# graphdeco-inria/editable-gaussian-reflections

Measured on AMD Instinct MI355X. Metric: Mrays/s fwd+bwd @1080p, 1M Gaussians, higher is better.
Workload: dtype f32; 1 GPU; BASELINE config C: synthetic dense-init room+spheres cloud, HEADLINE variant = init (literal dense-init opacity 0.1 (config.py:44): Kc ~ 22 per ray, bounces mostly die), N=1000000, 1920x1080, one training iteration: export + update_bvh + forward + backward + grad import, num_bounces=2, jitter on, reference default config; variant=init, gaussians=1000000, width=1920, height=1080, parallelism=image tiles x1 + 1 all-reduce of the launch's [22N] gradients, team_help=product default (on)

## Files before the change

editable-gaussian-reflections_amd/csrc/backward_chain.inc:

```
    const int lane = threadIdx.x & (EGR_WAVE - 1);
    const int wv = __builtin_amdgcn_readfirstlane((int)(threadIdx.x >> 6));
    __shared__ uint32_t gt_keys_all[TEAM][EGR_GT_SLOTS];
    __shared__ __attribute__((aligned(16))) float gt_vals_all[TEAM][EGR_GT_STRIDE * EGR_GT_SLOTS];
    __shared__ uint32_t gt_claim_all[TEAM][EGR_GT_SLOTS];
    __shared__ float4 stage_all[TEAM][4 * EGR_WAVE];
    __shared__ BwdTeamShared<TEAM> bteam;
    uint32_t *const gt_keys = gt_keys_all[wv], *const gt_claim = gt_claim_all[wv];
    float *const gt_vals = gt_vals_all[wv];
    float4 *const stage = stage_all[wv];
    if (threadIdx.x == 0) bteam.done = 0u;
    if (threadIdx.x < TEAM) bteam.ticket[threadIdx.x] = 0u, bteam.nitems[threadIdx.x] = 0u, bteam.finished[threadIdx.x] = 0u;
    uint32_t bepoch = 0u;
#define EGR_BQ_FLOATS (25 * EGR_WAVE)
    static_assert(EGR_GT_STRIDE * EGR_GT_SLOTS >= EGR_BQ_FLOATS, "the bounce queues must fit into the table");
    uint4 *bitems = reinterpret_cast<uint4 *>(gt_vals);
    float *bdl = gt_vals + 16 * EGR_WAVE;
    float *bray = gt_vals + 19 * EGR_WAVE;
    for (int s = lane; s < EGR_GT_SLOTS; s += EGR_WAVE) gt_keys[s] = EGR_GT_EMPTY;
    for (int s = lane; s < EGR_GT_STRIDE * EGR_GT_SLOTS; s += EGR_WAVE) gt_vals[s] = 0.0f;
    __syncthreads();
    const float exp_power = *v.cfg.exp_power;
    const float eps_scale_grad = *v.cfg.eps_scale_grad;
    const int num_bounces = min(*v.cfg.num_bounces, EGR_MAX_BOUNCES);
    const float view_size = BATCH ? 0.0f : tanf(*v.cam.vertical_fov_radians / 2.0f);
    uint32_t cur_q = blockIdx.x & 7u;
    uint32_t records = 0u;

    for (;;) {
        const uint32_t tq = wave_next_task(v.queues + 8 * EGR_QUEUE_STRIDE, BATCH ? v.num_tasks * v.batch_frames : v.num_tasks, cur_q, lane);
        if (tq == 0xFFFFFFFFu) break;
        EGR_TIMES(unsigned long long bw_t0 = 0ull, bw_t1 = 0ull; uint32_t bw_rows0 = 0u;) EGR_TIMES_IS(8, bw_t0 = __builtin_amdgcn_s_memrealtime();)
        bool table_dirty = false;
        {
            constexpr bool PRIMARY = true;
            const int step = 0;
            do {
#include "backward_task.inc"
// ... 10 lines not shown
            EGR_BWD_SYNC();
            for (int s = lane; s < EGR_BQ_FLOATS; s += EGR_WAVE) gt_vals[s] = 0.0f;
            EGR_BWD_SYNC();
        }
        EGR_TIMES_IS(8,
            const unsigned long long bw_t2 = __builtin_amdgcn_s_memrealtime();
            const uint32_t bt = v.bwd_order[tq];
            const TaskGeom btg = task_geom(v, BATCH ? batch_base_task(v, bt) : bt, lane);
            if (btg.inside) {
                if (lane == 0) v.stats.num_traversed_per_pixel[btg.pixel_id] = EGR_STAMP31(bw_t0), v.stats.num_accumulated_per_pixel[btg.pixel_id] = EGR_STAMP31(bw_t2);
                if (lane == 1) v.stats.num_traversed_per_pixel[btg.pixel_id] = EGR_STAMP31(bw_t1), v.stats.num_accumulated_per_pixel[btg.pixel_id] = (int32_t)bw_rows0;
            })
    }
    if constexpr (TEAM > 1) {
        if (lane == 0) atomicAdd(&bteam.done, 1u);
        records += bwd_team_help<TEAM>(v, exp_power, eps_scale_grad, bteam, gt_vals_all, stage, wv, lane);
    }
    if (lane == 0 && records) atomicAdd(v.control + CW_BUCKET_RECORDS, records);
```

editable-gaussian-reflections_amd/csrc/backward_task.inc:

```
        const uint32_t task = v.bwd_order[tq];
        uint32_t blk = v.task_last_block[(size_t)step * (BATCH ? v.num_tasks * v.batch_frames : v.num_tasks) + task];
        if (blk == 0xFFFFFFFFu) continue;
        uint32_t tb = task, bframe = 0u;
        if constexpr (BATCH) tb = batch_base_task(v, task), bframe = v.batch_frame0 + (task >> v.task_shift) % v.batch_frames;
        (void)bframe;
        const TaskGeom tg = task_geom(v, tb, lane);
        const StateRef S = state_of(v, task, lane);
        uint32_t steps_done = tg.inside ? f2u(S.ld(F_STEPS)) : 0u;
        uint32_t nhits = (tg.inside && (uint32_t)step < steps_done && blk != 0xFFFFFFFFu) ? f2u(S.ld(SF(step, S_NHITS))) : 0u;
        const uint32_t max_hits = wave_max_u32(nhits);
        if (max_hits == 0) continue;
        EGR_TIMES_IS(8, if (PRIMARY) bw_rows0 = max_hits;)

        f3 dL_rgb = mk3(0, 0, 0), dL_n = mk3(0, 0, 0), dL_f0 = mk3(0, 0, 0);
        float dL_depth = 0.0f, dL_rough = 0.0f;
        f3 ro = mk3(0, 0, 0), rd = mk3(0, 0, 1);
        f3 rem_rgb = mk3(0, 0, 0), rem_n = mk3(0, 0, 0), rem_f0 = mk3(0, 0, 0);
        float rem_depth = 0.0f, rem_rough = 0.0f, T_minus_Ttot = 0.0f;
        if (nhits > 0) {
            const uint32_t pid = tg.pixel_id;
            const float third = 1.0f / 3.0f;
            if (PRIMARY && BATCH) {
                f3 o_rgb = S.ld3(SF(0, S_RGB)), o_n = S.ld3(SF(0, S_NORMAL)), o_f0 = S.ld3(SF(0, S_F0));
                float o_depth = S.ld(SF(0, S_DEPTH)), o_rough = S.ld(SF(0, S_ROUGH));
// ... 34 lines not shown
                    const float *ts = v.fb.target_specular + 3 * (size_t)pid;
                    t_spec = mk3(ts[0], ts[1], ts[2]);
                }
                float down = powf(1.0f - S.ld(SF(step - 1, S_ROUGH)), EGR_ROUGHNESS_DOWNWEIGHT_GRAD_POWER);
                dL_rgb = (mk3(third * sign1(spec.x - t_spec.x), third * sign1(spec.y - t_spec.y), third * sign1(spec.z - t_spec.z)) *
                          *v.cfg.loss_weight_specular) * down;
                dL_rgb = dL_rgb * S.ld3(SF(step - 1, S_THR));
                ro = S.ld3(SF(step - 1, S_NEXT_O));
                rd = S.ld3(SF(step - 1, S_NEXT_D));
            }
            rem_rgb = S.ld3(SF(step, S_REM_RGB)), rem_n = S.ld3(SF(step, S_REM_NORMAL)), rem_f0 = S.ld3(SF(step, S_REM_F0));
            rem_depth = S.ld(SF(step, S_REM_DEPTH)), rem_rough = S.ld(SF(step, S_REM_ROUGH));
            T_minus_Ttot = S.ld(SF(step, S_T)) - S.ld(SF(step, S_TTOT));
        }

        auto hit_geometry = [&](uint32_t pos, const float4 &a2, const f3 &ro, const f3 &rd, float dL_dalpha, auto &gx) { hit_geometry_fn<true>(v, exp_power, eps_scale_grad, pos, a2, ro, rd, dL_dalpha, gx); };

        if constexpr (!PRIMARY) {
            table_dirty = true;
            bdl[lane] = dL_rgb.x, bdl[EGR_WAVE + lane] = dL_rgb.y, bdl[2 * EGR_WAVE + lane] = dL_rgb.z;
            bray[lane] = ro.x, bray[EGR_WAVE + lane] = ro.y, bray[2 * EGR_WAVE + lane] = ro.z, bray[3 * EGR_WAVE + lane] = rd.x, bray[4 * EGR_WAVE + lane] = rd.y, bray[5 * EGR_WAVE + lane] = rd.z;
            f3 prev_rgb = mk3(0, 0, 0), w_rgb = mk3(0, 0, 0);
            const uint32_t nblocks = (max_hits + EGR_HIT_BLOCK_ROWS - 1) / EGR_HIT_BLOCK_ROWS;
            EGR_BWD_SYNC();
            for (uint32_t b = nblocks; b-- > 0;) {
                const float4 *rows = v.hit_arena + (size_t)blk * (EGR_HIT_BLOCK_ROWS + 1) * EGR_WAVE;
                for (int chunk = EGR_HIT_BLOCK_ROWS / 4 - 1; chunk >= 0; chunk--) {
                    uint32_t nitems = 0u;
                    float4 rec4[4], a04[4];
#pragma unroll
                    for (int r4 = 0; r4 < 4; r4++) rec4[r4] = rows[(size_t)(1 + 4 * chunk + r4) * EGR_WAVE + lane];
// ... 29 lines not shown
                    EGR_BWD_SYNC();
                    const uint32_t nbatch = (nitems + (uint32_t)EGR_WAVE - 1u) / (uint32_t)EGR_WAVE;
                    if constexpr (TEAM > 1) {
                        if (lane == 0) {
                            lds_poke(&bteam.finished[wv], 0u);
                            lds_poke(&bteam.nitems[wv], nitems);
                            bepoch = (bepoch + 1u) & 0xFFFu;
                            lds_poke(&bteam.ticket[wv], (bepoch << 20) | (nbatch << 10));
                        }
                        for (;;) {
                            uint32_t tk = 0u;
                            if (lane == 0) tk = atomicAdd(&bteam.ticket[wv], 1u);
                            tk = uniform_u32(tk);
                            const uint32_t bi = tk & 0x3FFu;
                            if (bi >= nbatch) break;
                            records += bounce_batch(v, exp_power, eps_scale_grad, bitems, bdl, bray, bi * (uint32_t)EGR_WAVE, nitems, stage, lane);
                            if (lane == 0) atomicAdd(&bteam.finished[wv], 1u);
                        }
                        while (uniform_u32(lds_peek(&bteam.finished[wv])) < nbatch) __builtin_amdgcn_s_sleep(1);
                    } else {
                        for (uint32_t bi = 0; bi < nbatch; bi++) records += bounce_batch(v, exp_power, eps_scale_grad, bitems, bdl, bray, bi * (uint32_t)EGR_WAVE, nitems, stage, lane);
                    }
                    EGR_BWD_SYNC();
                }
                blk = f2u(rows[0].x);
            }
            continue;
        }
        f3 prev_rgb = mk3(0, 0, 0), w_rgb = mk3(0, 0, 0), prev_n = mk3(0, 0, 0), w_n = mk3(0, 0, 0), prev_f0 = mk3(0, 0, 0), w_f0 = mk3(0, 0, 0);
        float prev_rough = 0, w_rough = 0, prev_depth = 0, w_depth = 0;
        const uint32_t nblocks = (max_hits + EGR_HIT_BLOCK_ROWS - 1) / EGR_HIT_BLOCK_ROWS;
        EGR_STATS(unsigned long long bt_math = 0ull, bt_table = 0ull, bt_wide = 0ull, bt_rows = 0ull;)
        for (uint32_t b = nblocks; b-- > 0;) {
            const float4 *rows = v.hit_arena + (size_t)blk * (EGR_HIT_BLOCK_ROWS + 1) * EGR_WAVE;
            int pf_row = -1;
            float4 rec_pf = make_float4(0.f, 0.f, 0.f, 0.f);
// ... 54 lines not shown
                    dL_dalpha += tmp2 * dot(rem_f0, dL_f0);
                    dL_dalpha += tmp2 * (rem_rough * dL_rough);
                    dL_dalpha += tmp2 * (rem_depth * dL_depth);

                    hit_geometry(pos, a2, ro, rd, dL_dalpha, gx);
                    gx[PC_RGB] = d_rgb.x, gx[PC_RGB + 1] = d_rgb.y, gx[PC_RGB + 2] = d_rgb.z, gx[PC_WEIGHT] = weight;
                    gx[PC_NORMAL] = d_n.x, gx[PC_NORMAL + 1] = d_n.y, gx[PC_NORMAL + 2] = d_n.z;
                    gx[PC_F0] = d_f0.x, gx[PC_F0 + 1] = d_f0.y, gx[PC_F0 + 2] = d_f0.z, gx[PC_ROUGH] = d_rough;
                    EGR_STATS(bt1 = __builtin_amdgcn_s_memtime();)
                    dpos = pos;
                    want = primary_presum(pos, gx, lane);
                }
                direct = primary_table_add(v, want, dpos, gx, gt_keys, gt_vals, gt_claim, stage, lane, records);
                EGR_STATS(const unsigned long long bt2 = __builtin_amdgcn_s_memtime(); bt_math += bt1 - bt0; bt_table += bt2 - bt1;)
                if (__ballot(direct) != 0ull) {
                    float lo[15];
#pragma unroll
                    for (int c = 0; c < 15; c++) lo[c] = gx[c];
                    wide_add_wave<REC_PRIMARY_A>(v, direct, dpos, lo, stage);
                    float hi[15];
#pragma unroll
                    for (int c = 0; c < 15; c++) hi[c] = (15 + c < EGR_GT_COMPS) ? gx[(15 + c < EGR_GT_COMPS) ? 15 + c : 0] : 0.0f;
                    wide_add_wave<REC_PRIMARY_Q>(v, direct, dpos, hi, stage);
                    records += 2u * (uint32_t)__popcll(__ballot(direct));
                }
                EGR_STATS(bt_wide += __builtin_amdgcn_s_memtime() - bt2;)
            }
            blk = f2u(rows[0].x);
        }
        EGR_STATS(const unsigned long long bt3 = __builtin_amdgcn_s_memtime();)
        records += grad_table_flush(v, gt_keys, gt_vals, stage, lane);
        EGR_STATS(if (lane == 0) {
            unsigned long long *d = diag64(v.control, DG_BWD_MATH_CYC, !PRIMARY);
            atomicAdd(d, bt_math), atomicAdd(d + 1, bt_table), atomicAdd(d + 2, bt_wide), atomicAdd(d + 3, __builtin_amdgcn_s_memtime() - bt3), atomicAdd(d + 4, bt_rows);
        })
```

editable-gaussian-reflections_amd/csrc/trace.hip:

```cpp
#include <algorithm>
#include <cstdio>
#include <cstdlib>
#include <type_traits>
#include <utility>
#include <vector>

#define EGR_CONTRACT_AFTER_EPILOGUE
#include "egr_diag.hpp"
#include "egr_epilogue.hpp"

#ifndef EGR_GPOP
#define EGR_GPOP 5
#endif
#define EGR_WALK_MAX_LEAVES (8 * EGR_GPOP * EGR_WIDTH)
#define EGR_LBUF (64 + 2 * EGR_WALK_MAX_LEAVES)
#ifndef EGR_FPOP
#define EGR_FPOP 2
#endif
#ifndef EGR_PSTK
#define EGR_PSTK 512
#endif

namespace {

// ... 515 lines not shown
template <bool CUBE, int TEAM> __global__ void __launch_bounds__(EGR_WAVE * TEAM) __attribute__((amdgpu_waves_per_eu(EGR_FWD_WAVES, EGR_FWD_WAVES))) k_forward_batch(DeviceView v) {
    constexpr bool GRADS = false, BATCH = true;
#include "forward_chain.inc"
}
template <bool CUBE, int TEAM> __global__ void __launch_bounds__(EGR_WAVE * TEAM) __attribute__((amdgpu_waves_per_eu(EGR_FWD_WAVES, EGR_FWD_WAVES))) k_forward_batch_grads(DeviceView v) {
    constexpr bool GRADS = true, BATCH = true;
#include "forward_chain.inc"
}

#ifndef EGR_GT_SLOTS
#define EGR_GT_SLOTS 80
#endif
#define EGR_GT_COMPS 21
#define EGR_GT_STRIDE 21
#define EGR_GT_EMPTY 0xFFFFFFFFu
enum : int { GC_OPA = 0, GC_SCALE = 1, GC_MEAN = 4, GC_ROT = 7, GC_RGB = 11, GC_WEIGHT = 14, GC_NORMAL = 15, GC_F0 = 18, GC_ROUGH = 21, GC_Q = 22 };
enum : int { PC_OPA = 0, PC_MEAN = 1, PC_RGB = 4, PC_WEIGHT = 7, PC_NORMAL = 8, PC_F0 = 11, PC_ROUGH = 14, PC_Q = 15 };
enum : int { REC_BOUNCE = 0, REC_PRIMARY_A = 1, REC_PRIMARY_Q = 2 };
#define EGR_ROW_STRIDE 32
#define EGR_BWD_SYNC() wave_sync()

template <int REC> EGR_DI void wide_add_wave(const DeviceView &v, bool ok, uint32_t pos, const float (&r)[15], float4 *stage) {
    const int lane = threadIdx.x & (EGR_WAVE - 1);
    uint32_t cell = 0u;
    if constexpr (REC == REC_PRIMARY_A) {
        constexpr int cells[15] = {GC_OPA, GC_MEAN, GC_MEAN + 1, GC_MEAN + 2, GC_RGB, GC_RGB + 1, GC_RGB + 2, GC_WEIGHT, GC_NORMAL, GC_NORMAL + 1, GC_NORMAL + 2, GC_F0, GC_F0 + 1, GC_F0 + 2, GC_ROUGH};
#pragma unroll
        for (int i = 0; i < 15; i++) cell = (lane & 15) == i + 1 ? (uint32_t)cells[i] : cell;
    } else {
        cell = (REC == REC_PRIMARY_Q ? (uint32_t)GC_Q : 0u) + (uint32_t)((lane & 15) - 1);
    }
    if (ok) {
        stage[4 * lane + 0] = make_float4(u2f(pos), r[0], r[1], r[2]);
        stage[4 * lane + 1] = make_float4(r[3], r[4], r[5], r[6]);
        stage[4 * lane + 2] = make_float4(r[7], r[8], r[9], r[10]);
        stage[4 * lane + 3] = make_float4(r[11], r[12], r[13], r[14]);
    }
    const unsigned long long okm = __ballot(ok);
    EGR_BWD_SYNC();
    const float *sf = reinterpret_cast<const float *>(stage);
#pragma unroll 4
    for (int pass = 0; pass < 16; pass++) {
        const int src = 4 * pass + (lane >> 4), c = lane & 15;
        if (((okm >> (4 * pass)) & 0xFull) == 0ull) continue;
        const float x = sf[16 * src + c];
        const uint32_t p = f2u(sf[16 * src]);
        if (((okm >> src) & 1ull) && c != 0 && (REC != REC_PRIMARY_Q || c <= 6) && x != 0.0f) atomicAdd(v.grad_rows + (size_t)p * EGR_ROW_STRIDE + cell, x);
    }
    EGR_BWD_SYNC();
}

EGR_DI uint32_t grad_table_flush(const DeviceView &v, uint32_t *gt_keys, float *gt_vals, float4 *stage, int lane) {
    uint32_t sent = 0u;
    EGR_BWD_SYNC();
    for (int s0 = 0; s0 < EGR_GT_SLOTS; s0 += EGR_WAVE) {
        const int s = min(s0 + lane, EGR_GT_SLOTS - 1);
        const bool in_table = s0 + lane < EGR_GT_SLOTS;
        const uint32_t pos = in_table ? gt_keys[s] : EGR_GT_EMPTY;
        const bool valid = pos != EGR_GT_EMPTY;
        if (in_table) gt_keys[s] = EGR_GT_EMPTY;
        float lo[15], hi[15];
#pragma unroll
        for (int c = 0; c < 15; c++) {
            lo[c] = valid ? gt_vals[s * EGR_GT_STRIDE + c] : 0.0f;
            if (valid) gt_vals[s * EGR_GT_STRIDE + c] = 0.0f;
        }
#pragma unroll
        for (int c = 0; c < 15; c++) {
            hi[c] = 0.0f;
            if (15 + c < EGR_GT_COMPS) {
                hi[c] = valid ? gt_vals[s * EGR_GT_STRIDE + 15 + c] : 0.0f;
                if (valid) gt_vals[s * EGR_GT_STRIDE + 15 + c] = 0.0f;
            }
        }
        if (__ballot(valid) == 0ull) continue;
        wide_add_wave<REC_PRIMARY_A>(v, valid, pos, lo, stage);
        wide_add_wave<REC_PRIMARY_Q>(v, valid, pos, hi, stage);
        sent += 2u * (uint32_t)__popcll(__ballot(valid));
    }
    EGR_BWD_SYNC();
    return sent;
}

EGR_DI bool primary_presum(const uint32_t pos, float (&gx)[EGR_GT_COMPS], const int lane) {
    bool mine = true;
    {
        const unsigned long long em = __ballot(true);
#define EGR_FETCH_DPP(x, ctrl) __builtin_amdgcn_update_dpp(0, (int)(x), ctrl, 0xF, 0xF, false)
#define EGR_FETCH_SWZ(x, pat) __builtin_amdgcn_ds_swizzle((int)(x), pat)
#define EGR_FETCH_X32(x, unused) __shfl_xor((int)(x), 32)
#define EGR_FETCH_DPP4(x, unused) __builtin_amdgcn_update_dpp(0, __builtin_amdgcn_update_dpp(0, (int)(x), 0x141, 0xF, 0xF, false), 0x1B, 0xF, 0xF, false)
#define EGR_COMBINE(d, FETCH, arg)                                                                            \
// ... 45 lines not shown
        const bool win = pending && gt_claim[slot] == (uint32_t)lane;
        if (win) {
            float *cell = gt_vals + slot * EGR_GT_STRIDE;
            float cur[EGR_GT_COMPS];
#pragma unroll
            for (int c = 0; c < EGR_GT_COMPS; c++) cur[c] = cell[c];
#pragma unroll
            for (int c = 0; c < EGR_GT_COMPS; c++) cell[c] = cur[c] + gx[c];
            pending = false;
        }
        EGR_BWD_SYNC();
    }
    return want && !found;
}

template <class T> EGR_DI T chain_rcp(T b) {
    if constexpr (sizeof(T) == sizeof(float)) return egr_rcp_refined(b);
    else return T(1) / b;
}
template <class T> EGR_DI T chain_div(T a, T b, T r) {
    if constexpr (sizeof(T) == sizeof(float)) return egr_div_rn(a, b, r);
    else return a / b;
}
template <class T> EGR_DI T chain_sqrt(T x) {
    if constexpr (sizeof(T) == sizeof(float)) return egr_sqrt_rn(x);
    else return sqrt(x);
}
template <class T> struct ChainVec { T x, y, z; };
template <class T> EGR_DI void scale_rot_chain(const float4 &M0, const float4 &M1, const float4 &M2, const float4 &qu, const float sigma, const float eps, const ChainVec<T> &dl2w0,
                                               const ChainVec<T> &dl2w1, const ChainVec<T> &dl2w2, T (&d_scale)[3], T (&d_rot)[4]) {
    const T scaling_factor = sigma, eps_scale_grad = eps;
    const ChainVec<T> scaling = {T(M0.w), T(M1.w), T(M2.w)};
    const ChainVec<T> den = {scaling.x * scaling_factor + eps_scale_grad, scaling.y * scaling_factor + eps_scale_grad, scaling.z * scaling_factor + eps_scale_grad};
    const ChainVec<T> rden = {chain_rcp(den.x), chain_rcp(den.y), chain_rcp(den.z)};
    auto div3 = [&](const float4 &m) { return ChainVec<T>{chain_div(T(m.x), den.x, rden.x), chain_div(T(m.y), den.y, rden.y), chain_div(T(m.z), den.z, rden.z)}; };
    const ChainVec<T> rot_0 = div3(M0), rot_1 = div3(M1), rot_2 = div3(M2);
    d_scale[0] = (dl2w0.x * rot_0.x + dl2w1.x * rot_1.x + dl2w2.x * rot_2.x) * scaling.x;
    d_scale[1] = (dl2w0.y * rot_0.y + dl2w1.y * rot_1.y + dl2w2.y * rot_2.y) * scaling.y;
    d_scale[2] = (dl2w0.z * rot_0.z + dl2w1.z * rot_1.z + dl2w2.z * rot_2.z) * scaling.z;
    auto mul3 = [](const ChainVec<T> &a, const ChainVec<T> &b) { return ChainVec<T>{a.x * b.x, a.y * b.y, a.z * b.z}; };
    const ChainVec<T> dr0 = mul3(dl2w0, scaling), dr1 = mul3(dl2w1, scaling), dr2 = mul3(dl2w2, scaling);
    const T qr = qu.x, qx = qu.y, qy = qu.z, qz = qu.w;
    const T qn = chain_sqrt(qr * qr + qx * qx + qy * qy + qz * qz);
    const T rqn = chain_rcp(qn);
    const T r = chain_div(qr, qn, rqn), x = chain_div(qx, qn, rqn), y = chain_div(qy, qn, rqn), z = chain_div(qz, qn, rqn);
    const T dL_dr = T(2) * x * (dr2.y - dr1.z) + T(2) * y * (dr0.z - dr2.x) + T(2) * z * (dr1.x - dr0.y);
    const T dL_dx = T(-4) * x * (dr1.y + dr2.z) + T(2) * y * (dr0.y + dr1.x) + T(2) * z * (dr0.z + dr2.x) + T(2) * r * (dr2.y - dr1.z);
    const T dL_dy = T(2) * x * (dr0.y + dr1.x) - T(4) * y * (dr0.x + dr2.z) + T(2) * z * (dr1.z + dr2.y) + T(2) * r * (dr0.z - dr2.x);
    const T dL_dz = T(2) * x * (dr0.z + dr2.x) + T(2) * y * (dr1.z + dr2.y) - T(4) * z * (dr0.x + dr1.y) + T(2) * r * (dr1.x - dr0.y);
    const T dd = dL_dr * qr + dL_dx * qx + dL_dy * qy + dL_dz * qz;
    const T qn3 = qn * qn * qn;
    const T inv3 = chain_div(T(1), qn3, chain_rcp(qn3)), inv1 = chain_div(T(1), qn, rqn);
    d_rot[0] = dd * -qr * inv3 + dL_dr * inv1, d_rot[1] = dd * -qx * inv3 + dL_dx * inv1;
    d_rot[2] = dd * -qy * inv3 + dL_dy * inv1, d_rot[3] = dd * -qz * inv3 + dL_dz * inv1;
}

template <bool PRIMARY_HIT, class GX> EGR_DI void hit_geometry_fn(const DeviceView &v, const float exp_power, const float eps_scale_grad, uint32_t pos, const float4 &a2, const f3 &ro, const f3 &rd, float dL_dalpha, GX &gx) {
    const float opacity = a2.z, scaling_factor = a2.w;
    const float4 W0 = v.inst_w[4 * pos], W1 = v.inst_w[4 * pos + 1], W2 = v.inst_w[4 * pos + 2];
    float4 M0, M1, M2, qu;
    if constexpr (!PRIMARY_HIT) M0 = v.inst_m[4 * pos], M1 = v.inst_m[4 * pos + 1], M2 = v.inst_m[4 * pos + 2], qu = v.inst_m[4 * pos + 3];
    f3 lo, ld, dhat, u;
    float t_unused;
    bool behind_unused, outside_unused;
    candidate_geometry(W0, W1, W2, ro, rd, lo, ld, dhat, t_unused, u, behind_unused, outside_unused);
    const f3 local_hit = u * scaling_factor;
    const float sq_norm = dot(local_hit, local_hit);
    const float gaussval = egr_gaussian_sq(sq_norm, exp_power);

    float d_opacity = EGR_MAX_ALPHA * dL_dalpha * gaussval;
    d_opacity = d_opacity * opacity * (1.0f - opacity);
    const float dL_dgaussval = EGR_MAX_ALPHA * dL_dalpha * opacity;
    const float dL_dsq_norm = gaussval * pow_exp_m1(sq_norm, exp_power);
    const f3 dL_dx_local = (-local_hit * dL_dsq_norm) * dL_dgaussval;
    const f3 dL_dx_world = mk3(dot(mk3(W0.x, W1.x, W2.x), dL_dx_local), dot(mk3(W0.y, W1.y, W2.y), dL_dx_local),
                               dot(mk3(W0.z, W1.z, W2.z), dL_dx_local)) * scaling_factor;
    const f3 d_mean = -dL_dx_world;
    if constexpr (PRIMARY_HIT) {
        gx[PC_OPA] = d_opacity, gx[PC_MEAN] = d_mean.x, gx[PC_MEAN + 1] = d_mean.y, gx[PC_MEAN + 2] = d_mean.z;
        const f3 ql = -dL_dx_local * scaling_factor;
        gx[PC_Q] = ql.x * local_hit.x, gx[PC_Q + 1] = ql.x * local_hit.y, gx[PC_Q + 2] = ql.x * local_hit.z;
        gx[PC_Q + 3] = ql.y * local_hit.y, gx[PC_Q + 4] = ql.y * local_hit.z, gx[PC_Q + 5] = ql.z * local_hit.z;
    } else {
        const f3 dl2w0 = -dL_dx_world.x * local_hit, dl2w1 = -dL_dx_world.y * local_hit, dl2w2 = -dL_dx_world.z * local_hit;
        float d_scale[3], d_rot[4];
        scale_rot_chain<float>(M0, M1, M2, qu, scaling_factor, eps_scale_grad, {dl2w0.x, dl2w0.y, dl2w0.z}, {dl2w1.x, dl2w1.y, dl2w1.z}, {dl2w2.x, dl2w2.y, dl2w2.z}, d_scale, d_rot);
        gx[GC_OPA] = d_opacity, gx[GC_SCALE] = d_scale[0], gx[GC_SCALE + 1] = d_scale[1], gx[GC_SCALE + 2] = d_scale[2];
        gx[GC_MEAN] = d_mean.x, gx[GC_MEAN + 1] = d_mean.y, gx[GC_MEAN + 2] = d_mean.z;
        gx[GC_ROT] = d_rot[0], gx[GC_ROT + 1] = d_rot[1], gx[GC_ROT + 2] = d_rot[2], gx[GC_ROT + 3] = d_rot[3];
    }
}

EGR_DI uint32_t bounce_batch(const DeviceView &v, const float exp_power, const float eps_scale_grad, const uint4 *bitems, const float *bdl, const float *bray, uint32_t i0, uint32_t nitems,
                             float4 *stage, int lane) {
    const bool valid = i0 + (uint32_t)lane < nitems;
    uint32_t dpos = 0;
    float gx[15];
#pragma unroll
    for (int c = 0; c < 15; c++) gx[c] = 0.0f;
    if (valid) {
        const uint4 item = bitems[i0 + (uint32_t)lane];
        const uint32_t ray = item.x, pos = item.z;
        const float weight = u2f(item.w);
        const float4 a2 = v.inst_w[4 * pos + 3];
        const f3 iro = mk3(bray[ray], bray[EGR_WAVE + ray], bray[2 * EGR_WAVE + ray]), ird = mk3(bray[3 * EGR_WAVE + ray], bray[4 * EGR_WAVE + ray], bray[5 * EGR_WAVE + ray]);
        hit_geometry_fn<false>(v, exp_power, eps_scale_grad, pos, a2, iro, ird, u2f(item.y), gx);
        gx[GC_RGB] = bdl[ray] * weight, gx[GC_RGB + 1] = bdl[EGR_WAVE + ray] * weight, gx[GC_RGB + 2] = bdl[2 * EGR_WAVE + ray] * weight;
        gx[GC_WEIGHT] = weight;
        dpos = pos;
    }
    wide_add_wave<REC_BOUNCE>(v, valid, dpos, gx, stage);
    return (uint32_t)__popcll(__ballot(valid));
}

#ifndef EGR_BWD_TEAM
#define EGR_BWD_TEAM 4
#endif
template <int TEAM> struct BwdTeamShared {
    uint32_t done;
    uint32_t ticket[TEAM], nitems[TEAM], finished[TEAM];
};

#ifndef EGR_BWD_WAVES
#define EGR_BWD_WAVES 3
#endif
#ifndef EGR_ORDER_BUCKETS
// ... 24 lines not shown
    __syncthreads();
    uint32_t start[EGR_ORDER_BUCKETS];
    uint32_t acc = 0u;
#pragma unroll
    for (int b = 0; b < EGR_ORDER_BUCKETS; b++) start[b] = acc + cnt[b][t], acc += cnt[b][256];
    for (uint32_t i = i0; i < i1; i++) {
        const uint32_t bk = bucket(v.task_cost[beg + i]);
        uint32_t at = 0u;
#pragma unroll
        for (int b = 0; b < EGR_ORDER_BUCKETS; b++)
            if ((uint32_t)b == bk) at = start[b]++;
        v.bwd_order[beg + at] = beg + i;
    }
}

template <int TEAM> EGR_DI uint32_t bwd_team_help(const DeviceView &v, const float exp_power, const float eps_scale_grad, BwdTeamShared<TEAM> &bteam, float (*gt_vals_all)[EGR_GT_STRIDE * EGR_GT_SLOTS],
                                                  float4 *stage, const int wv, const int lane) {
    uint32_t records = 0u;
    while (uniform_u32(lds_peek(&bteam.done)) < (uint32_t)TEAM) {
        bool any = false;
        for (int dlt = 1; dlt < TEAM; dlt++) {
            const int w = (wv + dlt) % TEAM;
            const uint32_t peek = uniform_u32(lds_peek(&bteam.ticket[w]));
            if ((peek & 0x3FFu) >= ((peek >> 10) & 0x3FFu)) continue;
            uint32_t tk = 0u;
            if (lane == 0) tk = atomicAdd(&bteam.ticket[w], 1u);
            tk = uniform_u32(tk);
            const uint32_t bi = tk & 0x3FFu, nbatch = (tk >> 10) & 0x3FFu;
            if (bi >= nbatch) continue;
            const uint32_t nitems = uniform_u32(lds_peek(&bteam.nitems[w]));
            const uint4 *bitems = reinterpret_cast<const uint4 *>(gt_vals_all[w]);
            records += bounce_batch(v, exp_power, eps_scale_grad, bitems, gt_vals_all[w] + 16 * EGR_WAVE, gt_vals_all[w] + 19 * EGR_WAVE, bi * (uint32_t)EGR_WAVE, nitems, stage, lane);
            if (lane == 0) atomicAdd(&bteam.finished[w], 1u);
            any = true;
        }
        if (!any) __builtin_amdgcn_s_sleep(2);
    }
    return records;
}

template <int TEAM> __global__ void __launch_bounds__(EGR_WAVE * TEAM) __attribute__((amdgpu_waves_per_eu(EGR_BWD_WAVES, EGR_BWD_WAVES))) k_backward_chain(DeviceView v) {
    constexpr bool BATCH = false;
#include "backward_chain.inc"
}
template <int TEAM> __global__ void __launch_bounds__(EGR_WAVE * TEAM) __attribute__((amdgpu_waves_per_eu(EGR_BWD_WAVES, EGR_BWD_WAVES))) k_backward_batch(DeviceView v) {
    constexpr bool BATCH = true;
#include "backward_chain.inc"
// ... 7 lines not shown
    float x[EGR_ROW_STRIDE];
    uint32_t any = 0, any_l = 0;
#pragma unroll
    for (int q = 0; q < EGR_ROW_STRIDE / 4; q++) {
        const float4 r = row[q];
        x[4 * q] = r.x, x[4 * q + 1] = r.y, x[4 * q + 2] = r.z, x[4 * q + 3] = r.w;
        any |= (f2u(r.x) | f2u(r.y) | f2u(r.z) | f2u(r.w)) << 1;
    }
    if (!OVERWRITE && any == 0) return;
    if (any != 0) {
#pragma unroll
        for (int q = 0; q < EGR_ROW_STRIDE / 4; q++) row[q] = make_float4(0.f, 0.f, 0.f, 0.f);
    }
#pragma unroll
    for (int c = 0; c < 6; c++) any_l |= f2u(x[GC_Q + c]) << 1;
    if (any_l != 0) {
        const float4 M0 = v.inst_m[4 * pos], M1 = v.inst_m[4 * pos + 1], M2 = v.inst_m[4 * pos + 2], qu = v.inst_m[4 * pos + 3];
        const float4 W0 = v.inst_w[4 * pos], W1 = v.inst_w[4 * pos + 1], W2 = v.inst_w[4 * pos + 2];
        const float scaling_factor = v.inst_w[4 * pos + 3].w;
        const double q00 = x[GC_Q], q01 = x[GC_Q + 1], q02 = x[GC_Q + 2], q11 = x[GC_Q + 3], q12 = x[GC_Q + 4], q22 = x[GC_Q + 5];
        auto dl2w_of = [&](double w0, double w1, double w2) { return ChainVec<double>{w0 * q00 + w1 * q01 + w2 * q02, w0 * q01 + w1 * q11 + w2 * q12, w0 * q02 + w1 * q12 + w2 * q22}; };
        double d_scale[3], d_rot[4];
        scale_rot_chain<double>(M0, M1, M2, qu, scaling_factor, *v.cfg.eps_scale_grad, dl2w_of(W0.x, W1.x, W2.x), dl2w_of(W0.y, W1.y, W2.y), dl2w_of(W0.z, W1.z, W2.z), d_scale, d_rot);
#pragma unroll
        for (int a = 0; a < 3; a++) x[GC_SCALE + a] = (float)((double)x[GC_SCALE + a] + d_scale[a]);
#pragma unroll
        for (int a = 0; a < 4; a++) x[GC_ROT + a] = (float)((double)x[GC_ROT + a] + d_rot[a]);
    }
    const egr_gaussians &g = v.g;
    auto put = [](float *p, float val) {
        if (OVERWRITE) *p = val;
        else *p += val;
    };
    put(g.dL_dopacity + gid, x[GC_OPA]);
#pragma unroll
    for (int a = 0; a < 3; a++) {
        put(g.dL_dscale + 3 * gid + a, x[GC_SCALE + a]), put(g.dL_dmean + 3 * gid + a, x[GC_MEAN + a]), put(g.dL_drgb + 3 * gid + a, x[GC_RGB + a]);
        put(g.dL_dnormal + 3 * gid + a, x[GC_NORMAL + a]), put(g.dL_df0 + 3 * gid + a, x[GC_F0 + a]);
    }
#pragma unroll
    for (int a = 0; a < 4; a++) put(g.dL_drotation + 4 * gid + a, x[GC_ROT + a]);
    put(g.dL_droughness + gid, x[GC_ROUGH]);
    put(g.total_weight + gid, x[GC_WEIGHT]);
}

__global__ void __launch_bounds__(EGR_WAVE) k_finish(DeviceView v) {
    const int lane = threadIdx.x;
    const bool accumulate = *v.cfg.accumulate_samples != 0;
    const float cnt = accumulate ? (float)(*v.fb.accumulated_sample_count + 1) : 1.0f;
    const size_t P = v.num_pixels;
    for (uint32_t task = blockIdx.x; task < v.num_tasks; task += gridDim.x) {
        const TaskGeom tg = task_geom(v, task, lane);
        if (!tg.inside) continue;
        const StateRef S = state_of(v, task, lane);
        const uint32_t steps = f2u(S.ld(F_STEPS));
        f3 final = mk3(0, 0, 0);
// ... 597 lines not shown
```

Measured before the change: 456.0 Mrays/s.

## Defer bounce-hit scale/rotation chain to gather via moment records and re-lay row

```diff
diff --git a/editable-gaussian-reflections_amd/csrc/backward_chain.inc b/editable-gaussian-reflections_amd/csrc/backward_chain.inc
--- a/editable-gaussian-reflections_amd/csrc/backward_chain.inc
+++ b/editable-gaussian-reflections_amd/csrc/backward_chain.inc
@@ -20,7 +20,6 @@
     for (int s = lane; s < EGR_GT_STRIDE * EGR_GT_SLOTS; s += EGR_WAVE) gt_vals[s] = 0.0f;
     __syncthreads();
     const float exp_power = *v.cfg.exp_power;
-    const float eps_scale_grad = *v.cfg.eps_scale_grad;
     const int num_bounces = min(*v.cfg.num_bounces, EGR_MAX_BOUNCES);
     const float view_size = BATCH ? 0.0f : tanf(*v.cam.vertical_fov_radians / 2.0f);
     uint32_t cur_q = blockIdx.x & 7u;
@@ -61,6 +60,6 @@
     }
     if constexpr (TEAM > 1) {
         if (lane == 0) atomicAdd(&bteam.done, 1u);
-        records += bwd_team_help<TEAM>(v, exp_power, eps_scale_grad, bteam, gt_vals_all, stage, wv, lane);
+        records += bwd_team_help<TEAM>(v, exp_power, bteam, gt_vals_all, stage, wv, lane);
     }
     if (lane == 0 && records) atomicAdd(v.control + CW_BUCKET_RECORDS, records);
diff --git a/editable-gaussian-reflections_amd/csrc/backward_task.inc b/editable-gaussian-reflections_amd/csrc/backward_task.inc
--- a/editable-gaussian-reflections_amd/csrc/backward_task.inc
+++ b/editable-gaussian-reflections_amd/csrc/backward_task.inc
@@ -72,7 +72,7 @@
             T_minus_Ttot = S.ld(SF(step, S_T)) - S.ld(SF(step, S_TTOT));
         }
 
-        auto hit_geometry = [&](uint32_t pos, const float4 &a2, const f3 &ro, const f3 &rd, float dL_dalpha, auto &gx) { hit_geometry_fn<true>(v, exp_power, eps_scale_grad, pos, a2, ro, rd, dL_dalpha, gx); };
+        auto hit_geometry = [&](uint32_t pos, const float4 &a2, const f3 &ro, const f3 &rd, float dL_dalpha, auto &gx) { hit_geometry_fn(v, exp_power, pos, a2, ro, rd, dL_dalpha, gx); };
 
         if constexpr (!PRIMARY) {
             table_dirty = true;
@@ -132,12 +132,12 @@
                             tk = uniform_u32(tk);
                             const uint32_t bi = tk & 0x3FFu;
                             if (bi >= nbatch) break;
-                            records += bounce_batch(v, exp_power, eps_scale_grad, bitems, bdl, bray, bi * (uint32_t)EGR_WAVE, nitems, stage, lane);
+                            records += bounce_batch(v, exp_power, bitems, bdl, bray, bi * (uint32_t)EGR_WAVE, nitems, stage, lane);
                             if (lane == 0) atomicAdd(&bteam.finished[wv], 1u);
                         }
                         while (uniform_u32(lds_peek(&bteam.finished[wv])) < nbatch) __builtin_amdgcn_s_sleep(1);
                     } else {
-                        for (uint32_t bi = 0; bi < nbatch; bi++) records += bounce_batch(v, exp_power, eps_scale_grad, bitems, bdl, bray, bi * (uint32_t)EGR_WAVE, nitems, stage, lane);
+                        for (uint32_t bi = 0; bi < nbatch; bi++) records += bounce_batch(v, exp_power, bitems, bdl, bray, bi * (uint32_t)EGR_WAVE, nitems, stage, lane);
                     }
                     EGR_BWD_SYNC();
                 }
@@ -222,14 +222,13 @@
                 direct = primary_table_add(v, want, dpos, gx, gt_keys, gt_vals, gt_claim, stage, lane, records);
                 EGR_STATS(const unsigned long long bt2 = __builtin_amdgcn_s_memtime(); bt_math += bt1 - bt0; bt_table += bt2 - bt1;)
                 if (__ballot(direct) != 0ull) {
-                    float lo[15];
-#pragma unroll
-                    for (int c = 0; c < 15; c++) lo[c] = gx[c];
-                    wide_add_wave<REC_PRIMARY_A>(v, direct, dpos, lo, stage);
-                    float hi[15];
-#pragma unroll
-                    for (int c = 0; c < 15; c++) hi[c] = (15 + c < EGR_GT_COMPS) ? gx[(15 + c < EGR_GT_COMPS) ? 15 + c : 0] : 0.0f;
-                    wide_add_wave<REC_PRIMARY_Q>(v, direct, dpos, hi, stage);
+                    float lo[EGR_REC0_COMPS], hi[EGR_REC1_COMPS];
+#pragma unroll
+                    for (int c = 0; c < EGR_REC0_COMPS; c++) lo[c] = gx[c];
+#pragma unroll
+                    for (int c = 0; c < EGR_REC1_COMPS; c++) hi[c] = gx[EGR_REC0_COMPS + c];
+                    wide_add_wave<EGR_REC0_CELL>(v, direct, dpos, lo, stage);
+                    wide_add_wave<EGR_REC1_CELL>(v, direct, dpos, hi, stage);
                     records += 2u * (uint32_t)__popcll(__ballot(direct));
                 }
                 EGR_STATS(bt_wide += __builtin_amdgcn_s_memtime() - bt2;)
diff --git a/editable-gaussian-reflections_amd/csrc/trace.hip b/editable-gaussian-reflections_amd/csrc/trace.hip
--- a/editable-gaussian-reflections_amd/csrc/trace.hip
+++ b/editable-gaussian-reflections_amd/csrc/trace.hip
@@ -553,27 +553,27 @@
 #define EGR_GT_COMPS 21
 #define EGR_GT_STRIDE 21
 #define EGR_GT_EMPTY 0xFFFFFFFFu
-enum : int { GC_OPA = 0, GC_SCALE = 1, GC_MEAN = 4, GC_ROT = 7, GC_RGB = 11, GC_WEIGHT = 14, GC_NORMAL = 15, GC_F0 = 18, GC_ROUGH = 21, GC_Q = 22 };
-enum : int { PC_OPA = 0, PC_MEAN = 1, PC_RGB = 4, PC_WEIGHT = 7, PC_NORMAL = 8, PC_F0 = 11, PC_ROUGH = 14, PC_Q = 15 };
-enum : int { REC_BOUNCE = 0, REC_PRIMARY_A = 1, REC_PRIMARY_Q = 2 };
+enum : int { GC_OPA = 0, GC_MEAN = 1, GC_RGB = 4, GC_WEIGHT = 7, GC_Q = 8, GC_NORMAL = 16, GC_F0 = 19, GC_ROUGH = 22 };
+enum : int { PC_OPA = 0, PC_MEAN = 1, PC_RGB = 4, PC_WEIGHT = 7, PC_Q = 8, PC_NORMAL = 14, PC_F0 = 17, PC_ROUGH = 20 };
+#define EGR_REC0_CELL 0
+#define EGR_REC0_COMPS 14
+#define EGR_REC1_CELL 16
+#define EGR_REC1_COMPS 7
+static_assert(EGR_REC0_COMPS + EGR_REC1_COMPS == EGR_GT_COMPS && PC_NORMAL == EGR_REC0_COMPS && GC_NORMAL == EGR_REC1_CELL, "the table's components are the two records, in order");
 #define EGR_ROW_STRIDE 32
 #define EGR_BWD_SYNC() wave_sync()
 
-template <int REC> EGR_DI void wide_add_wave(const DeviceView &v, bool ok, uint32_t pos, const float (&r)[15], float4 *stage) {
+template <int CELL, int N> EGR_DI void wide_add_wave(const DeviceView &v, bool ok, uint32_t pos, const float (&r)[N], float4 *stage) {
+    static_assert(N >= 1 && N <= 15, "a record is its row index and up to 15 values: 16 lanes");
+    static_assert(CELL >= 0 && CELL / 16 == (CELL + N - 1) / 16 && CELL + N <= EGR_ROW_STRIDE, "a record's cells lie in ONE 64-B segment of the row");
     const int lane = threadIdx.x & (EGR_WAVE - 1);
-    uint32_t cell = 0u;
-    if constexpr (REC == REC_PRIMARY_A) {
-        constexpr int cells[15] = {GC_OPA, GC_MEAN, GC_MEAN + 1, GC_MEAN + 2, GC_RGB, GC_RGB + 1, GC_RGB + 2, GC_WEIGHT, GC_NORMAL, GC_NORMAL + 1, GC_NORMAL + 2, GC_F0, GC_F0 + 1, GC_F0 + 2, GC_ROUGH};
-#pragma unroll
-        for (int i = 0; i < 15; i++) cell = (lane & 15) == i + 1 ? (uint32_t)cells[i] : cell;
-    } else {
-        cell = (REC == REC_PRIMARY_Q ? (uint32_t)GC_Q : 0u) + (uint32_t)((lane & 15) - 1);
-    }
+    const uint32_t cell = (uint32_t)CELL + (uint32_t)((lane & 15) - 1);
     if (ok) {
-        stage[4 * lane + 0] = make_float4(u2f(pos), r[0], r[1], r[2]);
-        stage[4 * lane + 1] = make_float4(r[3], r[4], r[5], r[6]);
-        stage[4 * lane + 2] = make_float4(r[7], r[8], r[9], r[10]);
-        stage[4 * lane + 3] = make_float4(r[11], r[12], r[13], r[14]);
+        auto rv = [&](int i) { return i < N ? r[i < N ? i : 0] : 0.0f; };
+        stage[4 * lane + 0] = make_float4(u2f(pos), rv(0), rv(1), rv(2));
+        if (N > 3) stage[4 * lane + 1] = make_float4(rv(3), rv(4), rv(5), rv(6));
+        if (N > 7) stage[4 * lane + 2] = make_float4(rv(7), rv(8), rv(9), rv(10));
+        if (N > 11) stage[4 * lane + 3] = make_float4(rv(11), rv(12), rv(13), rv(14));
     }
     const unsigned long long okm = __ballot(ok);
     EGR_BWD_SYNC();
@@ -584,7 +584,7 @@
         if (((okm >> (4 * pass)) & 0xFull) == 0ull) continue;
         const float x = sf[16 * src + c];
         const uint32_t p = f2u(sf[16 * src]);
-        if (((okm >> src) & 1ull) && c != 0 && (REC != REC_PRIMARY_Q || c <= 6) && x != 0.0f) atomicAdd(v.grad_rows + (size_t)p * EGR_ROW_STRIDE + cell, x);
+        if (((okm >> src) & 1ull) && c != 0 && c <= N && x != 0.0f) atomicAdd(v.grad_rows + (size_t)p * EGR_ROW_STRIDE + cell, x);
     }
     EGR_BWD_SYNC();
 }
@@ -598,23 +598,20 @@
         const uint32_t pos = in_table ? gt_keys[s] : EGR_GT_EMPTY;
         const bool valid = pos != EGR_GT_EMPTY;
         if (in_table) gt_keys[s] = EGR_GT_EMPTY;
-        float lo[15], hi[15];
-#pragma unroll
-        for (int c = 0; c < 15; c++) {
+        float lo[EGR_REC0_COMPS], hi[EGR_REC1_COMPS];
+#pragma unroll
+        for (int c = 0; c < EGR_REC0_COMPS; c++) {
             lo[c] = valid ? gt_vals[s * EGR_GT_STRIDE + c] : 0.0f;
             if (valid) gt_vals[s * EGR_GT_STRIDE + c] = 0.0f;
         }
 #pragma unroll
-        for (int c = 0; c < 15; c++) {
-            hi[c] = 0.0f;
-            if (15 + c < EGR_GT_COMPS) {
-                hi[c] = valid ? gt_vals[s * EGR_GT_STRIDE + 15 + c] : 0.0f;
-                if (valid) gt_vals[s * EGR_GT_STRIDE + 15 + c] = 0.0f;
-            }
+        for (int c = 0; c < EGR_REC1_COMPS; c++) {
+            hi[c] = valid ? gt_vals[s * EGR_GT_STRIDE + EGR_REC0_COMPS + c] : 0.0f;
+            if (valid) gt_vals[s * EGR_GT_STRIDE + EGR_REC0_COMPS + c] = 0.0f;
         }
         if (__ballot(valid) == 0ull) continue;
-        wide_add_wave<REC_PRIMARY_A>(v, valid, pos, lo, stage);
-        wide_add_wave<REC_PRIMARY_Q>(v, valid, pos, hi, stage);
+        wide_add_wave<EGR_REC0_CELL>(v, valid, pos, lo, stage);
+        wide_add_wave<EGR_REC1_CELL>(v, valid, pos, hi, stage);
         sent += 2u * (uint32_t)__popcll(__ballot(valid));
     }
     EGR_BWD_SYNC();
@@ -690,52 +687,37 @@
     return want && !found;
 }
 
-template <class T> EGR_DI T chain_rcp(T b) {
-    if constexpr (sizeof(T) == sizeof(float)) return egr_rcp_refined(b);
-    else return T(1) / b;
-}
-template <class T> EGR_DI T chain_div(T a, T b, T r) {
-    if constexpr (sizeof(T) == sizeof(float)) return egr_div_rn(a, b, r);
-    else return a / b;
-}
-template <class T> EGR_DI T chain_sqrt(T x) {
-    if constexpr (sizeof(T) == sizeof(float)) return egr_sqrt_rn(x);
-    else return sqrt(x);
-}
-template <class T> struct ChainVec { T x, y, z; };
-template <class T> EGR_DI void scale_rot_chain(const float4 &M0, const float4 &M1, const float4 &M2, const float4 &qu, const float sigma, const float eps, const ChainVec<T> &dl2w0,
-                                               const ChainVec<T> &dl2w1, const ChainVec<T> &dl2w2, T (&d_scale)[3], T (&d_rot)[4]) {
+struct ChainVec { double x, y, z; };
+EGR_DI void scale_rot_chain(const float4 &M0, const float4 &M1, const float4 &M2, const float4 &qu, const float sigma, const float eps, const ChainVec &dl2w0, const ChainVec &dl2w1,
+                            const ChainVec &dl2w2, double (&d_scale)[3], double (&d_rot)[4]) {
+    using T = double;
     const T scaling_factor = sigma, eps_scale_grad = eps;
-    const ChainVec<T> scaling = {T(M0.w), T(M1.w), T(M2.w)};
-    const ChainVec<T> den = {scaling.x * scaling_factor + eps_scale_grad, scaling.y * scaling_factor + eps_scale_grad, scaling.z * scaling_factor + eps_scale_grad};
-    const ChainVec<T> rden = {chain_rcp(den.x), chain_rcp(den.y), chain_rcp(den.z)};
-    auto div3 = [&](const float4 &m) { return ChainVec<T>{chain_div(T(m.x), den.x, rden.x), chain_div(T(m.y), den.y, rden.y), chain_div(T(m.z), den.z, rden.z)}; };
-    const ChainVec<T> rot_0 = div3(M0), rot_1 = div3(M1), rot_2 = div3(M2);
+    const ChainVec scaling = {T(M0.w), T(M1.w), T(M2.w)};
+    const ChainVec den = {scaling.x * scaling_factor + eps_scale_grad, scaling.y * scaling_factor + eps_scale_grad, scaling.z * scaling_factor + eps_scale_grad};
+    auto div3 = [&](const float4 &m) { return ChainVec{T(m.x) / den.x, T(m.y) / den.y, T(m.z) / den.z}; };
+    const ChainVec rot_0 = div3(M0), rot_1 = div3(M1), rot_2 = div3(M2);
     d_scale[0] = (dl2w0.x * rot_0.x + dl2w1.x * rot_1.x + dl2w2.x * rot_2.x) * scaling.x;
     d_scale[1] = (dl2w0.y * rot_0.y + dl2w1.y * rot_1.y + dl2w2.y * rot_2.y) * scaling.y;
     d_scale[2] = (dl2w0.z * rot_0.z + dl2w1.z * rot_1.z + dl2w2.z * rot_2.z) * scaling.z;
-    auto mul3 = [](const ChainVec<T> &a, const ChainVec<T> &b) { return ChainVec<T>{a.x * b.x, a.y * b.y, a.z * b.z}; };
-    const ChainVec<T> dr0 = mul3(dl2w0, scaling), dr1 = mul3(dl2w1, scaling), dr2 = mul3(dl2w2, scaling);
+    auto mul3 = [](const ChainVec &a, const ChainVec &b) { return ChainVec{a.x * b.x, a.y * b.y, a.z * b.z}; };
+    const ChainVec dr0 = mul3(dl2w0, scaling), dr1 = mul3(dl2w1, scaling), dr2 = mul3(dl2w2, scaling);
     const T qr = qu.x, qx = qu.y, qy = qu.z, qz = qu.w;
-    const T qn = chain_sqrt(qr * qr + qx * qx + qy * qy + qz * qz);
-    const T rqn = chain_rcp(qn);
-    const T r = chain_div(qr, qn, rqn), x = chain_div(qx, qn, rqn), y = chain_div(qy, qn, rqn), z = chain_div(qz, qn, rqn);
+    const T qn = sqrt(qr * qr + qx * qx + qy * qy + qz * qz);
+    const T r = qr / qn, x = qx / qn, y = qy / qn, z = qz / qn;
     const T dL_dr = T(2) * x * (dr2.y - dr1.z) + T(2) * y * (dr0.z - dr2.x) + T(2) * z * (dr1.x - dr0.y);
     const T dL_dx = T(-4) * x * (dr1.y + dr2.z) + T(2) * y * (dr0.y + dr1.x) + T(2) * z * (dr0.z + dr2.x) + T(2) * r * (dr2.y - dr1.z);
     const T dL_dy = T(2) * x * (dr0.y + dr1.x) - T(4) * y * (dr0.x + dr2.z) + T(2) * z * (dr1.z + dr2.y) + T(2) * r * (dr0.z - dr2.x);
     const T dL_dz = T(2) * x * (dr0.z + dr2.x) + T(2) * y * (dr1.z + dr2.y) - T(4) * z * (dr0.x + dr1.y) + T(2) * r * (dr1.x - dr0.y);
     const T dd = dL_dr * qr + dL_dx * qx + dL_dy * qy + dL_dz * qz;
     const T qn3 = qn * qn * qn;
-    const T inv3 = chain_div(T(1), qn3, chain_rcp(qn3)), inv1 = chain_div(T(1), qn, rqn);
+    const T inv3 = T(1) / qn3, inv1 = T(1) / qn;
     d_rot[0] = dd * -qr * inv3 + dL_dr * inv1, d_rot[1] = dd * -qx * inv3 + dL_dx * inv1;
     d_rot[2] = dd * -qy * inv3 + dL_dy * inv1, d_rot[3] = dd * -qz * inv3 + dL_dz * inv1;
 }
 
-template <bool PRIMARY_HIT, class GX> EGR_DI void hit_geometry_fn(const DeviceView &v, const float exp_power, const float eps_scale_grad, uint32_t pos, const float4 &a2, const f3 &ro, const f3 &rd, float dL_dalpha, GX &gx) {
+template <class GX> EGR_DI void hit_geometry_fn(const DeviceView &v, const float exp_power, uint32_t pos, const float4 &a2, const f3 &ro, const f3 &rd, float dL_dalpha, GX &gx) {
     const float opacity = a2.z, scaling_factor = a2.w;
     const float4 W0 = v.inst_w[4 * pos], W1 = v.inst_w[4 * pos + 1], W2 = v.inst_w[4 * pos + 2];
-    float4 M0, M1, M2, qu;
-    if constexpr (!PRIMARY_HIT) M0 = v.inst_m[4 * pos], M1 = v.inst_m[4 * pos + 1], M2 = v.inst_m[4 * pos + 2], qu = v.inst_m[4 * pos + 3];
     f3 lo, ld, dhat, u;
     float t_unused;
     bool behind_unused, outside_unused;
@@ -752,40 +734,31 @@
     const f3 dL_dx_world = mk3(dot(mk3(W0.x, W1.x, W2.x), dL_dx_local), dot(mk3(W0.y, W1.y, W2.y), dL_dx_local),
                                dot(mk3(W0.z, W1.z, W2.z), dL_dx_local)) * scaling_factor;
     const f3 d_mean = -dL_dx_world;
-    if constexpr (PRIMARY_HIT) {
-        gx[PC_OPA] = d_opacity, gx[PC_MEAN] = d_mean.x, gx[PC_MEAN + 1] = d_mean.y, gx[PC_MEAN + 2] = d_mean.z;
-        const f3 ql = -dL_dx_local * scaling_factor;
-        gx[PC_Q] = ql.x * local_hit.x, gx[PC_Q + 1] = ql.x * local_hit.y, gx[PC_Q + 2] = ql.x * local_hit.z;
-        gx[PC_Q + 3] = ql.y * local_hit.y, gx[PC_Q + 4] = ql.y * local_hit.z, gx[PC_Q + 5] = ql.z * local_hit.z;
-    } else {
-        const f3 dl2w0 = -dL_dx_world.x * local_hit, dl2w1 = -dL_dx_world.y * local_hit, dl2w2 = -dL_dx_world.z * local_hit;
-        float d_scale[3], d_rot[4];
-        scale_rot_chain<float>(M0, M1, M2, qu, scaling_factor, eps_scale_grad, {dl2w0.x, dl2w0.y, dl2w0.z}, {dl2w1.x, dl2w1.y, dl2w1.z}, {dl2w2.x, dl2w2.y, dl2w2.z}, d_scale, d_rot);
-        gx[GC_OPA] = d_opacity, gx[GC_SCALE] = d_scale[0], gx[GC_SCALE + 1] = d_scale[1], gx[GC_SCALE + 2] = d_scale[2];
-        gx[GC_MEAN] = d_mean.x, gx[GC_MEAN + 1] = d_mean.y, gx[GC_MEAN + 2] = d_mean.z;
-        gx[GC_ROT] = d_rot[0], gx[GC_ROT + 1] = d_rot[1], gx[GC_ROT + 2] = d_rot[2], gx[GC_ROT + 3] = d_rot[3];
-    }
-}
-
-EGR_DI uint32_t bounce_batch(const DeviceView &v, const float exp_power, const float eps_scale_grad, const uint4 *bitems, const float *bdl, const float *bray, uint32_t i0, uint32_t nitems,
-                             float4 *stage, int lane) {
+    gx[PC_OPA] = d_opacity, gx[PC_MEAN] = d_mean.x, gx[PC_MEAN + 1] = d_mean.y, gx[PC_MEAN + 2] = d_mean.z;
+    const f3 ql = -dL_dx_local * scaling_factor;
+    gx[PC_Q] = ql.x * local_hit.x, gx[PC_Q + 1] = ql.x * local_hit.y, gx[PC_Q + 2] = ql.x * local_hit.z;
+    gx[PC_Q + 3] = ql.y * local_hit.y, gx[PC_Q + 4] = ql.y * local_hit.z, gx[PC_Q + 5] = ql.z * local_hit.z;
+}
+
+EGR_DI uint32_t bounce_batch(const DeviceView &v, const float exp_power, const uint4 *bitems, const float *bdl, const float *bray, uint32_t i0, uint32_t nitems, float4 *stage, int lane) {
+    static_assert(PC_OPA == GC_OPA && PC_MEAN == GC_MEAN && PC_RGB == GC_RGB && PC_WEIGHT == GC_WEIGHT && PC_Q == GC_Q && GC_Q + 6 == EGR_REC0_COMPS, "components 0-13 of a hit are segment 0 of the row");
     const bool valid = i0 + (uint32_t)lane < nitems;
     uint32_t dpos = 0;
-    float gx[15];
-#pragma unroll
-    for (int c = 0; c < 15; c++) gx[c] = 0.0f;
+    float gx[EGR_REC0_COMPS];
+#pragma unroll
+    for (int c = 0; c < EGR_REC0_COMPS; c++) gx[c] = 0.0f;
     if (valid) {
         const uint4 item = bitems[i0 + (uint32_t)lane];
         const uint32_t ray = item.x, pos = item.z;
         const float weight = u2f(item.w);
         const float4 a2 = v.inst_w[4 * pos + 3];
         const f3 iro = mk3(bray[ray], bray[EGR_WAVE + ray], bray[2 * EGR_WAVE + ray]), ird = mk3(bray[3 * EGR_WAVE + ray], bray[4 * EGR_WAVE + ray], bray[5 * EGR_WAVE + ray]);
-        hit_geometry_fn<false>(v, exp_power, eps_scale_grad, pos, a2, iro, ird, u2f(item.y), gx);
+        hit_geometry_fn(v, exp_power, pos, a2, iro, ird, u2f(item.y), gx);
         gx[GC_RGB] = bdl[ray] * weight, gx[GC_RGB + 1] = bdl[EGR_WAVE + ray] * weight, gx[GC_RGB + 2] = bdl[2 * EGR_WAVE + ray] * weight;
         gx[GC_WEIGHT] = weight;
         dpos = pos;
     }
-    wide_add_wave<REC_BOUNCE>(v, valid, dpos, gx, stage);
+    wide_add_wave<EGR_REC0_CELL>(v, valid, dpos, gx, stage);
     return (uint32_t)__popcll(__ballot(valid));
 }
 
@@ -840,7 +813,7 @@
     }
 }
 
-template <int TEAM> EGR_DI uint32_t bwd_team_help(const DeviceView &v, const float exp_power, const float eps_scale_grad, BwdTeamShared<TEAM> &bteam, float (*gt_vals_all)[EGR_GT_STRIDE * EGR_GT_SLOTS],
+template <int TEAM> EGR_DI uint32_t bwd_team_help(const DeviceView &v, const float exp_power, BwdTeamShared<TEAM> &bteam, float (*gt_vals_all)[EGR_GT_STRIDE * EGR_GT_SLOTS],
                                                   float4 *stage, const int wv, const int lane) {
     uint32_t records = 0u;
     while (uniform_u32(lds_peek(&bteam.done)) < (uint32_t)TEAM) {
@@ -856,7 +829,7 @@
             if (bi >= nbatch) continue;
             const uint32_t nitems = uniform_u32(lds_peek(&bteam.nitems[w]));
             const uint4 *bitems = reinterpret_cast<const uint4 *>(gt_vals_all[w]);
-            records += bounce_batch(v, exp_power, eps_scale_grad, bitems, gt_vals_all[w] + 16 * EGR_WAVE, gt_vals_all[w] + 19 * EGR_WAVE, bi * (uint32_t)EGR_WAVE, nitems, stage, lane);
+            records += bounce_batch(v, exp_power, bitems, gt_vals_all[w] + 16 * EGR_WAVE, gt_vals_all[w] + 19 * EGR_WAVE, bi * (uint32_t)EGR_WAVE, nitems, stage, lane);
             if (lane == 0) atomicAdd(&bteam.finished[w], 1u);
             any = true;
         }
@@ -894,18 +867,19 @@
     }
 #pragma unroll
     for (int c = 0; c < 6; c++) any_l |= f2u(x[GC_Q + c]) << 1;
+    float d_scale[3] = {0.f, 0.f, 0.f}, d_rot[4] = {0.f, 0.f, 0.f, 0.f};
     if (any_l != 0) {
         const float4 M0 = v.inst_m[4 * pos], M1 = v.inst_m[4 * pos + 1], M2 = v.inst_m[4 * pos + 2], qu = v.inst_m[4 * pos + 3];
         const float4 W0 = v.inst_w[4 * pos], W1 = v.inst_w[4 * pos + 1], W2 = v.inst_w[4 * pos + 2];
         const float scaling_factor = v.inst_w[4 * pos + 3].w;
         const double q00 = x[GC_Q], q01 = x[GC_Q + 1], q02 = x[GC_Q + 2], q11 = x[GC_Q + 3], q12 = x[GC_Q + 4], q22 = x[GC_Q + 5];
-        auto dl2w_of = [&](double w0, double w1, double w2) { return ChainVec<double>{w0 * q00 + w1 * q01 + w2 * q02, w0 * q01 + w1 * q11 + w2 * q12, w0 * q02 + w1 * q12 + w2 * q22}; };
-        double d_scale[3], d_rot[4];
-        scale_rot_chain<double>(M0, M1, M2, qu, scaling_factor, *v.cfg.eps_scale_grad, dl2w_of(W0.x, W1.x, W2.x), dl2w_of(W0.y, W1.y, W2.y), dl2w_of(W0.z, W1.z, W2.z), d_scale, d_rot);
-#pragma unroll
-        for (int a = 0; a < 3; a++) x[GC_SCALE + a] = (float)((double)x[GC_SCALE + a] + d_scale[a]);
-#pragma unroll
-        for (int a = 0; a < 4; a++) x[GC_ROT + a] = (float)((double)x[GC_ROT + a] + d_rot[a]);
+        auto dl2w_of = [&](double w0, double w1, double w2) { return ChainVec{w0 * q00 + w1 * q01 + w2 * q02, w0 * q01 + w1 * q11 + w2 * q12, w0 * q02 + w1 * q12 + w2 * q22}; };
+        double ds[3], dr[4];
+        scale_rot_chain(M0, M1, M2, qu, scaling_factor, *v.cfg.eps_scale_grad, dl2w_of(W0.x, W1.x, W2.x), dl2w_of(W0.y, W1.y, W2.y), dl2w_of(W0.z, W1.z, W2.z), ds, dr);
+#pragma unroll
+        for (int a = 0; a < 3; a++) d_scale[a] = (float)ds[a];
+#pragma unroll
+        for (int a = 0; a < 4; a++) d_rot[a] = (float)dr[a];
     }
     const egr_gaussians &g = v.g;
     auto put = [](float *p, float val) {
@@ -915,11 +889,11 @@
     put(g.dL_dopacity + gid, x[GC_OPA]);
 #pragma unroll
     for (int a = 0; a < 3; a++) {
-        put(g.dL_dscale + 3 * gid + a, x[GC_SCALE + a]), put(g.dL_dmean + 3 * gid + a, x[GC_MEAN + a]), put(g.dL_drgb + 3 * gid + a, x[GC_RGB + a]);
+        put(g.dL_dscale + 3 * gid + a, d_scale[a]), put(g.dL_dmean + 3 * gid + a, x[GC_MEAN + a]), put(g.dL_drgb + 3 * gid + a, x[GC_RGB + a]);
         put(g.dL_dnormal + 3 * gid + a, x[GC_NORMAL + a]), put(g.dL_df0 + 3 * gid + a, x[GC_F0 + a]);
     }
 #pragma unroll
-    for (int a = 0; a < 4; a++) put(g.dL_drotation + 4 * gid + a, x[GC_ROT + a]);
+    for (int a = 0; a < 4; a++) put(g.dL_drotation + 4 * gid + a, d_rot[a]);
     put(g.dL_droughness + gid, x[GC_ROUGH]);
     put(g.total_weight + gid, x[GC_WEIGHT]);
 }
```

Result: faster. 461.0 Mrays/s, median of 6 (+1.1%).
